# mjmyt/drone_path_planning_python

Measured on AMD Instinct MI355X. Metric: minimum-snap trajectories/sec (N drones × M segments, order 7) at 1/2/4/8 MI355X, higher is better.
Workload: dtype f64

## Files before the change

drone_path_planning_python_amd/csrc/msnap_api.hip:

```cpp
#include <cstdarg>
#include <cstdio>
#include <cstdlib>
#include <cstring>
#include <initializer_list>
#include <new>

#include "msnap_internal.h"

namespace msnap {

int record_hip_error(msnap_ctx *ctx, hipError_t e, const char *what) {
  if (ctx) snprintf(ctx->hip_err, sizeof(ctx->hip_err), "%s: %s", what, hipGetErrorString(e));
  return MSNAP_EHIP;
}

int handover_form(const msnap_ctx *ctx, const void *ptr, const void *pos, int n, int n_samples) {
  if (!ptr) return 0;
  for (const auto &h : ctx->handover)
    if (h.ptr == ptr) return (h.pos == pos && h.n == n && h.s == n_samples) ? h.form : 0;
  return 0;
}

bool stream_is_capturing(const msnap_ctx *ctx) {
  hipStreamCaptureStatus st = hipStreamCaptureStatusNone;
// ... 42 lines not shown
  do {                                                            \
    const int rc__ = (check);                                     \
    if (rc__) return rc__ == msnap::kNoWork ? MSNAP_OK : rc__;    \
    MSNAP_HIP(ctx, hipSetDevice((ctx)->device));                  \
  } while (0)

struct Region {
  const void *in;
  void *out;
  size_t bytes;
};
static Region upload(const void *h, size_t bytes) { return {h, nullptr, bytes}; }
static Region download(void *h, size_t bytes) { return {nullptr, h, bytes}; }

struct DevPtr {
  void *p;
  template <class T>
  operator T *() const { return static_cast<T *>(p); }
};

template <size_t K, class Launch>
static int staged(msnap_ctx *ctx, const Region (&r)[K], Launch &&launch) {
  size_t off[K], total = 0;
  for (size_t k = 0; k < K; ++k) {
    off[k] = total;
    total += r[k].bytes ? (r[k].bytes + 255) & ~(size_t)255 : 256;
  }
  int rc = ensure(ctx, ctx->host_stage, total);
  if (rc) return rc;
  DevPtr d[K];
  for (size_t k = 0; k < K; ++k) {
    d[k].p = (char *)ctx->host_stage.p + off[k];
    if (r[k].in && r[k].bytes)
      MSNAP_HIP(ctx, hipMemcpyAsync(d[k].p, r[k].in, r[k].bytes, hipMemcpyHostToDevice, ctx->stream));
  }
  if ((rc = launch(d))) return rc;
  for (size_t k = 0; k < K; ++k)
    if (r[k].out && r[k].bytes)
      MSNAP_HIP(ctx, hipMemcpyAsync(r[k].out, d[k].p, r[k].bytes, hipMemcpyDeviceToHost, ctx->stream));
  MSNAP_HIP(ctx, hipStreamSynchronize(ctx->stream));
  return MSNAP_OK;
}

static size_t coef_bytes(const msnap_ctx *ctx, int n_drones, int n_seg) {
  return (size_t)n_drones * n_seg * 4 * (ctx->order + 1) * 8;
}
static size_t dur_bytes(int n_drones, int n_seg) { return (size_t)n_drones * n_seg * 8; }

struct OptionName {
  const char *name, *env;
};
static const OptionName kOptions[] = {
    {"solve_grid_waves", "MSNAP_SOLVE_GRID_WAVES"}, {"gemm_grid_waves", "MSNAP_GEMM_GRID_WAVES"},
    {"twist_max_drones", "MSNAP_TWIST_MAX_DRONES"}, {"no_twist", "MSNAP_NO_TWIST"},
    {"collide_waves_per_cu", "MSNAP_COLLIDE_WAVES_PER_CU"}, {"pipe_chunk_mb", "MSNAP_PIPE_CHUNK_MB"},
    {"collide_sample_parts", "MSNAP_COLLIDE_SAMPLE_PARTS"}, {"no_twin", "MSNAP_NO_TWIN"}, {"no_grid_sample", "MSNAP_NO_GRID_SAMPLE"}, {"gemm_stream_waves_per_cu", "MSNAP_GEMM_STREAM_WAVES_PER_CU"}, {"mesh_waves_per_cu", "MSNAP_MESH_WAVES_PER_CU"}, {"collide_no_cull", "MSNAP_COLLIDE_NO_CULL"}, {"collide_cull_min_drones", "MSNAP_COLLIDE_CULL_MIN_DRONES"}, {"collide_cull_mode", "MSNAP_COLLIDE_CULL_MODE"}, {"twin_max_drones", "MSNAP_TWIN_MAX_DRONES"},
};

void note_kernel(msnap_ctx *ctx, const char *fmt, ...) {
  va_list ap;
  va_start(ap, fmt);
  vsnprintf(ctx->last_kernel, sizeof(ctx->last_kernel), fmt, ap);
  va_end(ap);
}

static bool option_is_read_only(const char *name) { return !strncmp(name, "collide_last_", 13); }

static int *option_slot(msnap_ctx *ctx, const char *name) {
  if (!strcmp(name, "solve_grid_waves")) return &ctx->solve_grid_waves;
  if (!strcmp(name, "gemm_grid_waves")) return &ctx->gemm_grid_waves;
  if (!strcmp(name, "twist_max_drones")) return &ctx->twist_max_drones;
  if (!strcmp(name, "no_twist")) return &ctx->no_twist;
  if (!strcmp(name, "no_twin")) return &ctx->no_twin;
  if (!strcmp(name, "no_grid_sample")) return &ctx->no_grid_sample;
  if (!strcmp(name, "gemm_stream_waves_per_cu")) return &ctx->gemm_stream_waves_per_cu;
  if (!strcmp(name, "mesh_waves_per_cu")) return &ctx->mesh_waves_per_cu;
  if (!strcmp(name, "twin_max_drones")) return &ctx->twin_max_drones;
  if (!strcmp(name, "collide_waves_per_cu")) return &ctx->collide_waves_per_cu;
  if (!strcmp(name, "collide_sample_parts")) return &ctx->collide_sample_parts;
  if (!strcmp(name, "collide_no_sym")) return &ctx->collide_no_sym;
  if (!strcmp(name, "collide_no_cull")) return &ctx->collide_no_cull;
  if (!strcmp(name, "collide_cull_min_drones")) return &ctx->collide_cull_min_drones;
  if (!strcmp(name, "collide_cull_mode")) return &ctx->collide_cull_mode;
  if (!strcmp(name, "collide_last_cull")) return &ctx->collide_last_cull;
  if (!strcmp(name, "collide_last_shares")) return &ctx->collide_last_shares;
  if (!strcmp(name, "collide_last_sym")) return &ctx->collide_last_sym;
  if (!strcmp(name, "collide_last_handover")) return &ctx->collide_last_handover;
  if (!strcmp(name, "own_stream_priority")) return &ctx->own_stream_priority;
  return nullptr;
}

}

using namespace msnap;

extern "C" {

int msnap_version(void) { return MSNAP_VERSION_NUM; }

const char *msnap_strerror(int code) {
  switch (code) {
    case MSNAP_OK: return "ok";
    case MSNAP_EINVAL: return "invalid argument";
    case MSNAP_EHIP: return "HIP runtime error (see msnap_last_hip_error)";
    case MSNAP_EORDER: return "unsupported polynomial order (7 or 9)";
    case MSNAP_ESEGMENTS: return "segment count out of range for this context, or not the prepared grid's";
    case MSNAP_ENOMEM: return "out of memory";
    case MSNAP_ENODEVICE: return "no usable gfx950 device";
    case MSNAP_ENOGRID: return "no time grid prepared on this context (msnap_grid_prepare)";
    case MSNAP_ECAPTURE: return "a scratch buffer would have to grow during stream capture: run the call once outside the capture first";
    default: return "unknown msnap error";
  }
}

const char *msnap_last_hip_error(const msnap_ctx *ctx) { return ctx ? ctx->hip_err : ""; }

const char *msnap_last_kernel(const msnap_ctx *ctx) { return ctx ? ctx->last_kernel : ""; }

int msnap_create(msnap_ctx **out, int device_id, int order, int max_segments) {
  if (!out) return MSNAP_EINVAL;
  *out = nullptr;
  if (order != 7 && order != 9) return MSNAP_EORDER;
  if (max_segments < 1) return MSNAP_ESEGMENTS;
  int ndev = 0;
  if (hipGetDeviceCount(&ndev) != hipSuccess || ndev <= 0) return MSNAP_ENODEVICE;
// ... 70 lines not shown
  }
  if (bytes) *bytes = freed;
  return rc;
}

int msnap_set_stream(msnap_ctx *ctx, void *hip_stream) {
  if (!ctx) return MSNAP_EINVAL;
  ctx->stream = reinterpret_cast<hipStream_t>(hip_stream);
  return MSNAP_OK;
}

int msnap_use_own_stream(msnap_ctx *ctx) {
  if (!ctx) return MSNAP_EINVAL;
  ctx->stream = ctx->own_stream;
  return MSNAP_OK;
}

int msnap_set_option(msnap_ctx *ctx, const char *name, long value) {
  if (!ctx || !name || value < 0 || value > (1L << 30)) return MSNAP_EINVAL;
  if (!strcmp(name, "pipe_chunk_mb")) {
    ctx->pipe_chunk_bytes = (size_t)(value > 0 ? value : 64) << 20;
    return MSNAP_OK;
  }
  if (!strcmp(name, "own_stream_priority")) {
    if (value > 2) return MSNAP_EINVAL;
    MSNAP_HIP(ctx, hipSetDevice(ctx->device));
    int least = 0, greatest = 0;
    MSNAP_HIP(ctx, hipDeviceGetStreamPriorityRange(&least, &greatest));
    hipStream_t fresh = nullptr;
    MSNAP_HIP(ctx, hipStreamCreateWithPriority(&fresh, hipStreamNonBlocking,
                                               value == 1 ? least : value == 2 ? greatest : 0));
    const bool current = ctx->stream == ctx->own_stream;
    if (ctx->own_stream) {
      (void)hipStreamSynchronize(ctx->own_stream);
      (void)hipStreamDestroy(ctx->own_stream);
    }
    ctx->own_stream = fresh;
    if (current) ctx->stream = fresh;
    ctx->own_stream_priority = (int)value;
    return MSNAP_OK;
  }
  if (!strcmp(name, "mesh_count_tests")) {
    MSNAP_HIP(ctx, hipSetDevice(ctx->device));
    MSNAP_HIP(ctx, hipStreamSynchronize(ctx->stream));
    if (value && !ctx->mesh_tests) MSNAP_HIP(ctx, hipMalloc(&ctx->mesh_tests, 8));
    if (ctx->mesh_tests) MSNAP_HIP(ctx, hipMemset(ctx->mesh_tests, 0, 8));
    if (!value && ctx->mesh_tests) {
      (void)hipFree(ctx->mesh_tests);
      ctx->mesh_tests = nullptr;
    }
    return MSNAP_OK;
  }
  if (option_is_read_only(name)) return MSNAP_EINVAL;
  int *slot = option_slot(ctx, name);
  if (!slot) return MSNAP_EINVAL;
  *slot = (int)value;
  return MSNAP_OK;
}

int msnap_get_option(const msnap_ctx *ctx, const char *name, long *value) {
  if (!ctx || !name || !value) return MSNAP_EINVAL;
  if (!strcmp(name, "pipe_chunk_mb")) {
    *value = (long)(ctx->pipe_chunk_bytes >> 20);
    return MSNAP_OK;
  }
  if (!strcmp(name, "mesh_count_tests")) {
    unsigned long long n = 0;
    if (ctx->mesh_tests) {
      if (stream_is_capturing(ctx)) return MSNAP_ECAPTURE;
      if (hipSetDevice(ctx->device) != hipSuccess || hipStreamSynchronize(ctx->stream) != hipSuccess ||
          hipMemcpy(&n, ctx->mesh_tests, 8, hipMemcpyDeviceToHost) != hipSuccess)
        return MSNAP_EHIP;
    }
    *value = (long)n;
    return MSNAP_OK;
  }
  if (!strcmp(name, "collide_last_group_pairs") || !strcmp(name, "collide_last_survivors") ||
      !strcmp(name, "collide_last_by_groups") || !strcmp(name, "collide_last_pairs_evaluated")) {
    int32_t shares = ctx->collide_last_shares, groups = 0;
    const bool culled = ctx->collide_last_cull && ctx->collide_meta;
    if (culled) {
      if (stream_is_capturing(ctx)) return MSNAP_ECAPTURE;
      if (hipSetDevice(ctx->device) != hipSuccess || hipStreamSynchronize(ctx->stream) != hipSuccess ||
          hipMemcpy(&shares, ctx->collide_meta + MSNAP_COLLIDE_META_SHARES, sizeof shares, hipMemcpyDeviceToHost) != hipSuccess ||
          hipMemcpy(&groups, ctx->collide_meta + MSNAP_COLLIDE_META_GROUPS, sizeof groups, hipMemcpyDeviceToHost) != hipSuccess)
        return MSNAP_EHIP;
    }
    const bool by_groups = culled && (ctx->collide_last_by_groups == 1 || (ctx->collide_last_by_groups == 2 && groups <= (1 << 18)));
    if (!strcmp(name, "collide_last_group_pairs")) *value = groups;
    else if (!strcmp(name, "collide_last_survivors")) *value = shares;
    else if (!strcmp(name, "collide_last_by_groups")) *value = by_groups ? 1 : 0;
    else *value = !culled ? -1 : by_groups ? (long)groups * 64 : (long)shares * 1024;
    return MSNAP_OK;
  }
  const int *slot = option_slot(const_cast<msnap_ctx *>(ctx), name);
  if (!slot) return MSNAP_EINVAL;
  *value = *slot;
  return MSNAP_OK;
}

int msnap_host_alloc(void **ptr, size_t bytes) {
  if (!ptr) return MSNAP_EINVAL;
  *ptr = nullptr;
  if (bytes == 0) return MSNAP_OK;
  hipError_t e = hipHostMalloc(ptr, bytes, hipHostMallocDefault);
  if (e != hipSuccess) {
// ... 578 lines not shown
```

drone_path_planning_python_amd/csrc/msnap_internal.h:

```cpp
#pragma once

#include <hip/hip_runtime.h>
#include <stddef.h>
#include <stdint.h>

#include "../../include/msnap.h"

#define MSNAP_VERSION_NUM 300
#define MSNAP_COLLIDE_META_SHARES 128
#define MSNAP_COLLIDE_META_GROUPS 132

namespace msnap {

constexpr int kWave = 64;
constexpr int kAxes = 4;
constexpr int kDronesPerWave = 16;
constexpr size_t kMaxLdsBytes = 160 * 1024;

inline size_t solve_scratch_words(int khalf, int n_seg) {
  const size_t nu = (size_t)khalf - 1;
  const size_t M = (size_t)n_seg;
  const size_t knots = M > 0 ? M - 1 : 0;
  return 16 * M + 16 * nu * nu * knots + 64 * nu * knots;
}
inline size_t solve_input_words(int n_seg) { return (size_t)16 * (n_seg + 1) * 5; }

template <int N>
__device__ __forceinline__ void wait_vmcnt() {
  static_assert(N >= 0 && N < 64, "6-bit vmcnt field");
  asm volatile("s_waitcnt vmcnt(%0)" ::"n"(N) : "memory");
}

__device__ __forceinline__ void lds_barrier() { asm volatile("s_waitcnt lgkmcnt(0)\n\ts_barrier" ::: "memory"); }

struct DevBuf {
  void *p = nullptr;
  size_t cap = 0;
  bool in_graph = false;
};
struct RetiredBuf {
  void *p;
  size_t cap;
  RetiredBuf *next;
};

}

struct msnap_ctx {
  int device = 0;
  int order = 7;
  int khalf = 4;
  int max_segments = 0;
  int n_cu = 256;
  hipStream_t own_stream = nullptr;
  hipStream_t stream = nullptr;
  hipEvent_t ev0 = nullptr, ev1 = nullptr;
  msnap::DevBuf scratch;
  msnap::DevBuf host_stage;
  msnap::DevBuf collide_work;
  msnap::DevBuf limits_work;
  hipStream_t pipe_stream[2] = {nullptr, nullptr};
  hipEvent_t pipe_start = nullptr;
  msnap::DevBuf pipe[2][5];
  size_t pipe_chunk_bytes = 64u << 20;
  void *bounce = nullptr;
  size_t bounce_cap = 0;
  msnap::DevBuf grid_t, grid_wp, grid_op, grid_dur, grid_status, grid_frag;
  int grid_seg = 0;
  int grid_ready = 0;
  int no_twist = 0;
  int gemm_stream_waves_per_cu = 0;
  int no_grid_sample = 0;
  int no_twin = 0;
  int twin_max_drones = 0;
  int twist_max_drones = 0;
  int solve_grid_waves = 0;
  int gemm_grid_waves = 0;
  void *mesh_tests = nullptr;
  int collide_waves_per_cu = 0;
  int collide_sample_parts = 0;
  int collide_no_sym = 0;
  int collide_no_cull = 0;
  int collide_cull_mode = 0;
  int collide_cull_min_drones = 0;
  int collide_last_cull = 0;
  int collide_last_shares = 0;
  const int32_t *collide_meta = nullptr;
  int collide_last_by_groups = 0;
  int collide_last_n = 0;
  const void *blist_clean = nullptr;
  int blist_clean_n = 0;
  unsigned long long *cull_hint = nullptr;
  struct Handover {
    const void *ptr = nullptr;
    const void *pos = nullptr;
    int n = 0, s = 0, form = 0;
  } handover[8];
  int handover_next = 0;
  int collide_last_sym = 0;
  int collide_last_handover = 0;
  int mesh_waves_per_cu = 0;
  int own_stream_priority = 0;
  msnap::RetiredBuf *retired = nullptr;
  char hip_err[256] = {0};
  char last_kernel[96] = {0};
};

namespace msnap {

int record_hip_error(msnap_ctx *ctx, hipError_t e, const char *what);
int ensure(msnap_ctx *ctx, DevBuf &b, size_t bytes);
bool stream_is_capturing(const msnap_ctx *ctx);
int handover_form(const msnap_ctx *ctx, const void *ptr, const void *pos, int n, int n_samples);
bool collide_counts_by_groups(const msnap_ctx *ctx, int n_drones, int shares_surviving, int group_pairs_surviving);

void note_kernel(msnap_ctx *ctx, const char *fmt, ...) __attribute__((format(printf, 2, 3)));

#define MSNAP_HIP(ctx, call)                                         \
  do {                                                               \
    hipError_t e__ = (call);                                         \
    if (e__ != hipSuccess) return msnap::record_hip_error(ctx, e__, #call); \
  } while (0)

int launch_solve(msnap_ctx *ctx, int n_drones, int n_seg, const double *wp, const double *t,
                 int shared_times, double *coef, double *dur, int32_t *status);
int launch_pack(msnap_ctx *ctx, int n_drones, int n_seg, const double *coef, const double *dur,
                float *out);
int launch_formation_transform(msnap_ctx *ctx, int n_poses, int n_offsets, const double *rb_pose,
// ... 53 lines not shown
```

drone_path_planning_python_amd/csrc/msnap_solve.hip:

```cpp
#include "msnap_consts.h"
#include <cstdlib>

#include "msnap_internal.h"

namespace msnap {

__device__ __forceinline__ constexpr int sidx(int r, int c) {
  return r * (r + 1) / 2 + c;
}

__device__ __forceinline__ double rcp64(double v) {
  double r = __builtin_amdgcn_rcp(v);
  double e = __builtin_fma(-v, r, 1.0);
  r = __builtin_fma(r, e, r);
  e = __builtin_fma(-v, r, 1.0);
  r = __builtin_fma(r, e, r);
  return r;
}

__device__ __forceinline__ bool finite64(double v) { return __builtin_isfinite(v); }

template <int K>
struct Sweep {
  static constexpr int NU = K - 1;
// ... 247 lines not shown
        "s"(mask), "v"(keep[0]), "v"(keep[1]), "v"(keep[2]), "v"(keep[3]), "v"(keep[4]), "v"(keep[5]), "v"(keep[6]), \
        "v"(keep[7])                                                                                               \
      : "vcc")
template <int STAGE>
__device__ __forceinline__ void quad_stage(uint32_t (&a)[8], uint32_t (&b)[8], unsigned long long bit) {
  uint32_t na[8], nb[8];
  const unsigned long long nbit = ~bit;
  if constexpr (STAGE == 1) {
    MSNAP_QSTAGE("[1,0,3,2]", nb, a, b, bit);
    MSNAP_QSTAGE("[1,0,3,2]", na, b, a, nbit);
  } else {
    MSNAP_QSTAGE("[2,3,0,1]", nb, a, b, bit);
    MSNAP_QSTAGE("[2,3,0,1]", na, b, a, nbit);
  }
#pragma unroll
  for (int k = 0; k < 8; ++k) {
    a[k] = na[k];
    b[k] = nb[k];
  }
}
#undef MSNAP_QSTAGE
#undef MSNAP_QCND

__device__ __forceinline__ void store_quad8_at(double *__restrict__ blk, int a, const double (&c)[8], bool bad) {
  double p[8];
#pragma unroll
  for (int k = 0; k < 8; ++k) p[k] = c[k];
  if (__builtin_expect(__builtin_amdgcn_ballot_w64(bad) != 0, 0)) {
    asm volatile("" ::: "memory");
#pragma unroll
    for (int k = 0; k < 8; ++k) p[k] = bad ? __builtin_nan("") : p[k];
  }
  auto lo = [](double v) { return (uint32_t)__double2loint(v); };
  auto hi = [](double v) { return (uint32_t)__double2hiint(v); };
  uint32_t A[8] = {lo(p[0]), hi(p[0]), lo(p[1]), hi(p[1]), lo(p[4]), hi(p[4]), lo(p[5]), hi(p[5])};
  uint32_t B[8] = {lo(p[2]), hi(p[2]), lo(p[3]), hi(p[3]), lo(p[6]), hi(p[6]), lo(p[7]), hi(p[7])};
  quad_stage<1>(A, B, __builtin_amdgcn_ballot_w64((a & 1) != 0));
  uint32_t A2[8] = {A[0], A[1], A[2], A[3], B[0], B[1], B[2], B[3]};
  uint32_t B2[8] = {A[4], A[5], A[6], A[7], B[4], B[5], B[6], B[7]};
  quad_stage<2>(A2, B2, __builtin_amdgcn_ballot_w64((a & 2) != 0));
  uint4 *o = reinterpret_cast<uint4 *>(blk + a * 2);
  o[0] = make_uint4(A2[0], A2[1], A2[2], A2[3]);
  o[4] = make_uint4(A2[4], A2[5], A2[6], A2[7]);
  o[8] = make_uint4(B2[0], B2[1], B2[2], B2[3]);
  o[12] = make_uint4(B2[4], B2[5], B2[6], B2[7]);
}

__device__ __forceinline__ void store_segment_quad8(double *__restrict__ seg_base, size_t drone_stride,
                                                    int nvalid, int lane, const double (&c)[8], bool bad) {
  const int dl = lane >> 2;
  store_quad8_at(seg_base + (size_t)(dl < nvalid ? dl : nvalid - 1) * drone_stride, lane & 3, c, bad);
}

template <int MAXCNT = 0>
__device__ __forceinline__ void store_durations(const double *sTraw, int shared_times, int tpitch, int M,
                                                int nvalid, int lane, double *__restrict__ dur_tile) {
  const int cnt = nvalid * M;
  auto one = [&](int e) {
    if (e < cnt) {
      const int dl = e / M;
      const int i = e - dl * M;
      const double *lt = sTraw + (shared_times ? 0 : dl * tpitch);
      dur_tile[e] = lt[i + 1] - lt[i];
    }
  };
  if constexpr (MAXCNT > 0) {
#pragma unroll
    for (int e0 = 0; e0 < MAXCNT; e0 += kWave) one(e0 + lane);
  } else {
    for (int e0 = 0; e0 < cnt; e0 += kWave) one(e0 + lane);
  }
}

__device__ __forceinline__ int drone_status(bool nonfinite, bool badtime, bool singular) {
  int flags = (nonfinite ? 4 : 0) | (badtime ? 2 : 0) | (singular ? 1 : 0);
  flags |= __shfl_xor(flags, 1);
  flags |= __shfl_xor(flags, 2);
  return (flags & 4) ? MSNAP_ST_NONFINITE : (flags & 2) ? MSNAP_ST_TIMES : (flags & 1) ? MSNAP_ST_SINGULAR : MSNAP_ST_OK;
}

__device__ __forceinline__ void stage_inputs(const double *__restrict__ wp, const double *__restrict__ tt,
                                             int shared_times, int tile, int nvalid, int wpitch, int tpitch,
                                             double *sWraw, double *sTraw, int lane) {
  const double2 *wsrc = reinterpret_cast<const double2 *>(wp + (size_t)tile * kDronesPerWave * wpitch);
  double2 *wdst = reinterpret_cast<double2 *>(sWraw);
  const int wcnt = nvalid * wpitch / 2;
  const double *tsrc = shared_times ? tt : tt + (size_t)tile * kDronesPerWave * tpitch;
  const int tcnt = shared_times ? tpitch : nvalid * tpitch;
  constexpr int UW = 8, UT = 4;
  for (int e0 = 0, f0 = 0; e0 < wcnt || f0 < tcnt; e0 += UW * kWave, f0 += UT * kWave) {
    double2 vw[UW];
    double vt[UT];
#pragma unroll
    for (int u = 0; u < UW; ++u) {
      const int e = e0 + u * kWave + lane;
      vw[u] = wsrc[e < wcnt ? e : wcnt - 1];
    }
#pragma unroll
    for (int u = 0; u < UT; ++u) {
      const int f = f0 + u * kWave + lane;
      vt[u] = tsrc[f < tcnt ? f : tcnt - 1];
    }
#pragma unroll
    for (int u = 0; u < UW; ++u) asm volatile("" : "+v"(vw[u].x), "+v"(vw[u].y));
#pragma unroll
    for (int u = 0; u < UT; ++u) asm volatile("" : "+v"(vt[u]));
#pragma unroll
    for (int u = 0; u < UW; ++u) {
      const int e = e0 + u * kWave + lane;
      if (e < wcnt) wdst[e] = vw[u];
    }
#pragma unroll
    for (int u = 0; u < UT; ++u) {
      const int f = f0 + u * kWave + lane;
      if (f < tcnt) sTraw[f] = vt[u];
    }
  }
}

template <int MAXM>
struct StageRegs {
  static constexpr int UW = (MAXM + 2) / 2;
  static constexpr int UT = (MAXM + 4) / 4;
// ... 777 lines not shown
        __builtin_amdgcn_sched_barrier(0);
        const int nx = next < ntiles ? next : ntiles - 1;
        twin_stage_load<M>(wp, tt, shared_times, nx, tile_valid(nx), lane, pre);
      }
      const bool own = !kAsym || it <= nL || side != 0;
      double u[NU];
      if (it >= 1) {
        const double2 *gsl = reinterpret_cast<const double2 *>(sG + (it - 1) * kSlotWords + blk * kAxes);
#pragma unroll
        for (int r = 0; r < NU; ++r) {
          const double2 g01 = gsl[r * (kWave / 2)], g23 = gsl[r * (kWave / 2) + 1];
          double v = (it <= ZL) ? sZ[((it >= 1 ? it - 1 : 0) * NU + r) * kWave + lane] : zreg[it >= 1 ? it - 1 : 0][r];
          v = __builtin_fma(-g01.x, un[0], v);
          v = __builtin_fma(-g01.y, un[1], v);
          v = __builtin_fma(-g23.x, un[2], v);
          if constexpr (NU == 4) v = __builtin_fma(-g23.y, un[3], v);
          u[r] = v;
        }
      } else {
#pragma unroll
        for (int r = 0; r < NU; ++r) u[r] = zero_or_nan;
      }
      double ua[NU], ub[NU];
#pragma unroll
      for (int r = 0; r < NU; ++r) {
        ua[r] = side ? dsg[r] * un[r] : u[r];
        ub[r] = side ? dsg[r] * u[r] : un[r];
      }
      const double wa = side ? wreg[it + 1] : wreg[it];
      const double wb = side ? wreg[it] : wreg[it + 1];
      double xi = xreg[it];
      asm volatile("" : "+v"(xi));
      double c[NC];
      recover_segment<K>(wa, wb - wa, xi, ua, ub, c);
      if (side == 0 && it == 0 && t0 != 0.0) taylor_shift<NC>(c, -t0);
      if (own) {
        if constexpr (NC == 10) store_twin_coalesced(sTr, blkp, lane, plan, c);
        else store_quad8_at(blkp, a, c, false);
      }
      blkp += blkstep;
#pragma unroll
      for (int r = 0; r < NU; ++r) un[r] = own ? u[r] : un[r];
    }
  }
}

constexpr int kTwistDrones = 8;
constexpr int kTwistFenceHalf = 9;

#ifdef MSNAP_TOOLS_TIMELINE
__device__ unsigned long long g_timeline[1024 * 32];
#define MSNAP_TL(k)                                                                       \
  do {                                                                                    \
    const int it__ = (tl_tile - (int)blockIdx.x) / (int)gridDim.x;                        \
    if (lane == 0 && blockIdx.x < 1024 && it__ < 2) {                                     \
      g_timeline[blockIdx.x * 32 + 16 * it__ + 2 * (k)] = wall_clock64();                 \
      g_timeline[blockIdx.x * 32 + 16 * it__ + 2 * (k) + 1] = clock64();                  \
    }                                                                                     \
  } while (0)
#else
#define MSNAP_TL(k) do { } while (0)
#endif

template <int K, int MAXH, int M>
__global__ void __launch_bounds__(kWave)
solve_kernel_twist(const double *__restrict__ wp, const double *__restrict__ tt, int shared_times,
                   int N, double *__restrict__ coef, double *__restrict__ dur,
                   int32_t *__restrict__ status, int ntiles) {
  using SW = Sweep<K>;
  constexpr int NU = SW::NU, NC = SW::NC, NS = SW::NS;
  constexpr int nL = (M - 2) / 2, nR = (M - 2) - nL;
  static_assert(M >= 2 && MAXH == nR, "MAXH is the knot count of the longer side");
  constexpr int HA = MAXH > 0 ? MAXH : 1;

  extern __shared__ __attribute__((aligned(16))) double lds[];

  const int lane = threadIdx.x;
  const int a = lane & 3;
  const int side = (lane >> 2) & 1;
  const int dl = lane >> 3;
  constexpr int wpitch = (M + 1) * 4;
  constexpr int tpitch = M + 1;
  const int mside = side ? nR : nL;
  double *sWraw = lds;
  double *sTraw = sWraw + kTwistDrones * wpitch;
  double dsg[NU];
#pragma unroll
  for (int r = 0; r < NU; ++r) dsg[r] = (r & 1) ? 1.0 : -1.0;

  const int tile = blockIdx.x;
  (void)ntiles;
  {
#ifdef MSNAP_TOOLS_TIMELINE
    const int tl_tile = tile;
#endif
    MSNAP_TL(0);
    const int d_raw = tile * kTwistDrones + dl;
    const bool live = d_raw < N;
    const int d = live ? d_raw : N - 1;
    const int left = N - tile * kTwistDrones;
    const int nvalid = left < kTwistDrones ? left : kTwistDrones;

    {
      const double2 *wsrc = reinterpret_cast<const double2 *>(wp + (size_t)tile * kTwistDrones * wpitch);
      double2 *wdst = reinterpret_cast<double2 *>(sWraw);
      const int wcnt = nvalid * wpitch / 2;
      const double *tsrc = shared_times ? tt : tt + (size_t)tile * kTwistDrones * tpitch;
      const int tcnt = shared_times ? tpitch : nvalid * tpitch;
      constexpr int UW = (kTwistDrones * wpitch / 2 + kWave - 1) / kWave;
      constexpr int UT = (kTwistDrones * tpitch + kWave - 1) / kWave;
      double2 vw[UW];
      double vt[UT];
#pragma unroll
      for (int u = 0; u < UW; ++u) {
        const int e = u * kWave + lane;
        vw[u] = wsrc[e < wcnt ? e : wcnt - 1];
      }
#pragma unroll
      for (int u = 0; u < UT; ++u) {
        const int f = u * kWave + lane;
        vt[u] = tsrc[f < tcnt ? f : tcnt - 1];
      }
#pragma unroll
      for (int u = 0; u < UW; ++u) asm volatile("" : "+v"(vw[u].x), "+v"(vw[u].y));
#pragma unroll
      for (int u = 0; u < UT; ++u) asm volatile("" : "+v"(vt[u]));
#pragma unroll
      for (int u = 0; u < UW; ++u) {
        const int e = u * kWave + lane;
        if (e < wcnt) wdst[e] = vw[u];
      }
#pragma unroll
      for (int u = 0; u < UT; ++u) {
        const int f = u * kWave + lane;
        if (f < tcnt) sTraw[f] = vt[u];
      }
    }
    __syncthreads();
    MSNAP_TL(1);

    const int dloc = live ? dl : (N - 1 - tile * kTwistDrones);
    const double *lw = sWraw + dloc * wpitch + a;
    const double *lt = sTraw + (shared_times ? 0 : dloc * tpitch);
    auto Wown = [&](int i) -> double { return lw[(side ? M - i : i) * 4]; };
    auto Town = [&](int i) -> double {
      const int j = side ? M - 1 - i : i;
      return lt[j + 1] - lt[j];
    };

    constexpr bool kZReg = MAXH * NU < 3 * kTwistFenceHalf;
    double wreg[HA + 2], xreg[HA + 1], zreg[kZReg ? HA : 1][NU];
    double *sZ = sTraw + kTwistDrones * tpitch + lane;
    double Greg[HA][NU][NU];
    const double t0 = lt[0];
    wreg[0] = Wown(0);
    wreg[1] = Wown(1);
    const double T0 = Town(0);
    const double T0q = side ? T0 : T0 - t0;
    bool nonfinite = !(finite64(t0) & finite64(T0) & finite64(wreg[0]) & finite64(wreg[1]));
    bool badtime = !(T0 > 0.0) | !(T0q > 0.0) | (t0 < 0.0);
    xreg[0] = rcp64(T0q);
    SW sw;
    sw.init(xreg[0], wreg[1] - wreg[0]);

    double xpc[SW::PM + 1], dwc = 0.0;
    auto ahead = [&](int it, double (&xp)[SW::PM + 1], double &dw) {
      wreg[it + 1] = Wown(it + 1);
      const double Tit = Town(it);
      nonfinite |= !finite64(Tit) | !finite64(wreg[it + 1]);
      badtime |= !(Tit > 0.0);
      xreg[it] = rcp64(Tit);
      SW::powers(xreg[it], xp);
      dw = wreg[it + 1] - wreg[it];
    };
    if (MAXH >= 1) ahead(1, xpc, dwc);
    bool singular = false;
    auto knot_step = [&](int it) {
      double G[NU][NU], z[NU];
      typename SW::Knot k;
      SW::knot_geom_xp(xpc, dwc, sw.E, sw.re, k);
      const bool ok = sw.chain(k, G, z);
      singular |= !ok & (it <= mside);
#pragma unroll
      for (int e = 0; e < NS; ++e) sw.E[e] = k.E[e];
#pragma unroll
      for (int r = 0; r < NU; ++r) {
        sw.re[r] = k.re[r];
        if constexpr (kZReg) zreg[it - 1][r] = z[r];
        else sZ[((it - 1) * NU + r) * kWave] = z[r];
#pragma unroll
        for (int c = 0; c < NU; ++c) Greg[it - 1][r][c] = G[r][c];
      }
    };
#pragma unroll
    for (int it = 1; it <= MAXH; ++it) {
      if (it < MAXH) {
        double xpn[SW::PM + 1], dwn;
        ahead(it + 1, xpn, dwn);
        knot_step(it);
        dwc = dwn;
#pragma unroll
        for (int q = 0; q <= SW::PM; ++q) xpc[q] = xpn[q];
        if constexpr (MAXH * NU >= 3 * kTwistFenceHalf) __builtin_amdgcn_sched_barrier(0);
      } else if (nL == nR) {
        knot_step(it);
      } else {
        double E0[NS], G0[NS], r0[NU], z0[NU];
#pragma unroll
        for (int e = 0; e < NS; ++e) { E0[e] = sw.E[e]; G0[e] = sw.OtG[e]; }
#pragma unroll
        for (int r = 0; r < NU; ++r) { r0[r] = sw.re[r]; z0[r] = sw.Otz[r]; }
        knot_step(it);
#pragma unroll
        for (int e = 0; e < NS; ++e) { sw.E[e] = side ? sw.E[e] : E0[e]; sw.OtG[e] = side ? sw.OtG[e] : G0[e]; }
#pragma unroll
        for (int r = 0; r < NU; ++r) { sw.re[r] = side ? sw.re[r] : r0[r]; sw.Otz[r] = side ? sw.Otz[r] : z0[r]; }
      }
    }

    MSNAP_TL(2);
    double Sm[NS], um[NU];
#pragma unroll
    for (int r = 0; r < NU; ++r) {
      const double q = sw.re[r] + sw.Otz[r];
      um[r] = -q - dsg[r] * __shfl_xor(q, 4);
#pragma unroll
      for (int c = 0; c <= r; ++c) {
        const double p = sw.E[sidx(r, c)] - sw.OtG[sidx(r, c)];
        Sm[sidx(r, c)] = p + (dsg[r] * dsg[c]) * __shfl_xor(p, 4);
      }
    }
    {
      double dinv[NU];
      singular |= SW::ldl_factor(Sm, dinv);
      SW::ldl_solve(Sm, dinv, um);
    }

    const int gsh = lane & ~7;
    const bool f_nonfinite = ((__ballot(nonfinite) >> gsh) & 0xFFull) != 0;
    const bool f_time = ((__ballot(badtime) >> gsh) & 0xFFull) != 0;
    const bool f_sing = ((__ballot(singular) >> gsh) & 0xFFull) != 0;
    const int st = f_nonfinite ? MSNAP_ST_NONFINITE : f_time ? MSNAP_ST_TIMES : f_sing ? MSNAP_ST_SINGULAR : MSNAP_ST_OK;
    if (live && (lane & 7) == 0) status[d] = st;
    const bool bad = st != 0;

    MSNAP_TL(3);
    const double qnan = __builtin_nan("");
    const double zero_or_nan = bad ? qnan : 0.0;
#pragma unroll
    for (int i = 0; i < MAXH + 2; ++i) wreg[i] = bad ? qnan : wreg[i];
    double un[NU];
#pragma unroll
    for (int r = 0; r < NU; ++r) un[r] = bad ? qnan : um[r];
#pragma unroll
    for (int it = MAXH; it >= 0; --it) {
      if (it <= nL || side) {
        double u[NU];
        if (it >= 1) {
#pragma unroll
          for (int r = 0; r < NU; ++r) {
            double v;
            if constexpr (kZReg) v = zreg[it >= 1 ? it - 1 : 0][r];
            else v = sZ[((it >= 1 ? it - 1 : 0) * NU + r) * kWave];
#pragma unroll
            for (int c = 0; c < NU; ++c) v = __builtin_fma(-Greg[it >= 1 ? it - 1 : 0][r][c], un[c], v);
            u[r] = v;
          }
        } else {
#pragma unroll
          for (int r = 0; r < NU; ++r) u[r] = zero_or_nan;
        }
        double ua[NU], ub[NU];
#pragma unroll
        for (int r = 0; r < NU; ++r) {
          ua[r] = side ? dsg[r] * un[r] : u[r];
          ub[r] = side ? dsg[r] * u[r] : un[r];
        }
        const double wa = side ? wreg[it + 1] : wreg[it];
        const double wb = side ? wreg[it] : wreg[it + 1];
        double c[NC];
        recover_segment<K>(wa, wb - wa, xreg[it], ua, ub, c);
        if (side == 0 && it == 0 && t0 != 0.0) taylor_shift<NC>(c, -t0);
        const int seg = side ? M - 1 - it : it;
        {
          double *o = coef + (((size_t)d * M + seg) * 4 + a) * NC;
#pragma unroll
          for (int m = 0; m < NC; m += 2) *reinterpret_cast<double2 *>(o + m) = make_double2(c[m], c[m + 1]);
        }
#pragma unroll
        for (int r = 0; r < NU; ++r) un[r] = u[r];
      }
      if constexpr (MAXH * NU >= 3 * kTwistFenceHalf) __builtin_amdgcn_sched_barrier(0);
    }
    __builtin_amdgcn_sched_barrier(0);
    store_durations<kTwistDrones * M>(sTraw, shared_times, tpitch, M, nvalid, lane, dur + (size_t)tile * kTwistDrones * M);
    MSNAP_TL(4);
  }
}

constexpr int kTwistMaxSeg = 24;
constexpr int kTwistMaxSeg9 = 12;

constexpr int kTwinMaxSeg = 20;
constexpr int kTwinMaxSeg7 = 20;
constexpr int kRegMaxSeg = 10;
constexpr int kRegMaxSeg2 = 20;

template <int K>
static int launch_solve_k(msnap_ctx *ctx, int N, int M, const double *wp, const double *t, int shared,
                          double *coef, double *dur, int32_t *status) {
  const int ntiles = (N + kDronesPerWave - 1) / kDronesPerWave;
  const size_t tr_bytes = (size_t)K * kTrPitch * 16;
  const bool twin_ok = (M >= 4 && M <= (K == 5 ? kTwinMaxSeg : kTwinMaxSeg7) && !ctx->no_twin &&
                        (ctx->twin_max_drones > 0 ? N <= ctx->twin_max_drones
                                                   : (K == 5 || N <= ctx->n_cu * 256 || M > kRegMaxSeg)));
  const int twist_max = ctx->twist_max_drones > 0 ? ctx->twist_max_drones
                                                  : ctx->n_cu * (twin_ok ? 1 : 4) * kTwistDrones;
  if (M >= 2 && M <= (K == 4 ? kTwistMaxSeg : kTwistMaxSeg9) && N <= twist_max && !ctx->no_twist) {
    const int nt8 = (N + kTwistDrones - 1) / kTwistDrones;
    const int nR = (M - 2) - (M - 2) / 2;
    const size_t lds_bytes = ((size_t)kTwistDrones * (M + 1) * 5 + (size_t)64 * (K - 1) * nR) * sizeof(double);
#define MSNAP_TWIST_EXACT(MM)                                                                          \
  case MM:                                                                                             \
    note_kernel(ctx, "msnap::solve_kernel_twist<%d, %d, %d>", K, (MM - 2) - (MM - 2) / 2, MM);         \
    hipLaunchKernelGGL((solve_kernel_twist<K, (MM - 2) - (MM - 2) / 2, MM>), dim3(nt8), dim3(kWave),   \
                       lds_bytes, ctx->stream, wp, t, shared, N, coef, dur, status, nt8);             \
    break;
    if constexpr (K == 4) {
      switch (M) {
        MSNAP_TWIST_EXACT(2) MSNAP_TWIST_EXACT(3) MSNAP_TWIST_EXACT(4) MSNAP_TWIST_EXACT(5)
        MSNAP_TWIST_EXACT(6) MSNAP_TWIST_EXACT(7) MSNAP_TWIST_EXACT(8) MSNAP_TWIST_EXACT(9)
        MSNAP_TWIST_EXACT(10) MSNAP_TWIST_EXACT(11) MSNAP_TWIST_EXACT(12) MSNAP_TWIST_EXACT(13)
        MSNAP_TWIST_EXACT(14) MSNAP_TWIST_EXACT(15) MSNAP_TWIST_EXACT(16) MSNAP_TWIST_EXACT(17)
        MSNAP_TWIST_EXACT(18) MSNAP_TWIST_EXACT(19) MSNAP_TWIST_EXACT(20) MSNAP_TWIST_EXACT(21)
        MSNAP_TWIST_EXACT(22) MSNAP_TWIST_EXACT(23) MSNAP_TWIST_EXACT(24)
        default: return MSNAP_EINVAL;
      }
    } else {
      switch (M) {
        MSNAP_TWIST_EXACT(2) MSNAP_TWIST_EXACT(3) MSNAP_TWIST_EXACT(4) MSNAP_TWIST_EXACT(5)
        MSNAP_TWIST_EXACT(6) MSNAP_TWIST_EXACT(7) MSNAP_TWIST_EXACT(8) MSNAP_TWIST_EXACT(9)
        MSNAP_TWIST_EXACT(10) MSNAP_TWIST_EXACT(11) MSNAP_TWIST_EXACT(12)
        default: return MSNAP_EINVAL;
      }
    }
#undef MSNAP_TWIST_EXACT
    MSNAP_HIP(ctx, hipGetLastError());
    return MSNAP_OK;
  }
  if (twin_ok) {
    const int nt8 = (N + kTwinDrones - 1) / kTwinDrones;
    int grid = ctx->n_cu * 8 * 8;
    if (ctx->solve_grid_waves > 0) grid = ctx->solve_grid_waves;
    if (grid > nt8) grid = nt8;
#define MSNAP_TWIN(MM)                                                                                            \
  case MM:                                                                                                        \
    note_kernel(ctx, "msnap::solve_kernel_twin<%d, %d>", K, MM);                                                  \
    hipLaunchKernelGGL((solve_kernel_twin<K, MM>), dim3(grid), dim3(kWave), twin_lds_bytes(K, MM), ctx->stream,   \
                       wp, t, shared, N, coef, dur, status, nt8);                                                 \
    break;
    if constexpr (K == 5) {
      switch (M) {
        MSNAP_TWIN(4) MSNAP_TWIN(5) MSNAP_TWIN(6) MSNAP_TWIN(7) MSNAP_TWIN(8) MSNAP_TWIN(9) MSNAP_TWIN(10)
        MSNAP_TWIN(11) MSNAP_TWIN(12) MSNAP_TWIN(13) MSNAP_TWIN(14) MSNAP_TWIN(15) MSNAP_TWIN(16) MSNAP_TWIN(17)
        MSNAP_TWIN(18) MSNAP_TWIN(19) MSNAP_TWIN(20)
        default: return MSNAP_EINVAL;
      }
    } else {
      switch (M) {
        MSNAP_TWIN(4) MSNAP_TWIN(5) MSNAP_TWIN(6) MSNAP_TWIN(7) MSNAP_TWIN(8) MSNAP_TWIN(9) MSNAP_TWIN(10)
        MSNAP_TWIN(11) MSNAP_TWIN(12) MSNAP_TWIN(13) MSNAP_TWIN(14) MSNAP_TWIN(15) MSNAP_TWIN(16) MSNAP_TWIN(17)
        MSNAP_TWIN(18) MSNAP_TWIN(19) MSNAP_TWIN(20)
        default: return MSNAP_EINVAL;
      }
    }
#undef MSNAP_TWIN
    MSNAP_HIP(ctx, hipGetLastError());
    return MSNAP_OK;
  }
  if (M >= 2 && M <= kRegMaxSeg2) {
    const size_t nu = K - 1;
    const size_t in_bytes = solve_input_words(M) * sizeof(double);
    const size_t lds_bytes = (in_bytes > tr_bytes ? in_bytes : tr_bytes) +
                             16 * nu * nu * (size_t)(M > 2 ? M - 2 : 0) * sizeof(double);
    const bool two_per_simd = (K <= 4 && M <= kRegMaxSeg);
    int grid = ctx->n_cu * (two_per_simd ? 8 : 4) * 8;
    if (ctx->solve_grid_waves > 0) grid = ctx->solve_grid_waves;
    if (grid > ntiles) grid = ntiles;
    note_kernel(ctx, "msnap::solve_kernel_reg<%d, %d>", K, M <= kRegMaxSeg ? kRegMaxSeg : kRegMaxSeg2);
    if (M <= kRegMaxSeg)
      hipLaunchKernelGGL((solve_kernel_reg<K, kRegMaxSeg>), dim3(grid), dim3(kWave), lds_bytes, ctx->stream,
                         wp, t, shared, N, M, coef, dur, status, ntiles);
    else
      hipLaunchKernelGGL((solve_kernel_reg<K, kRegMaxSeg2>), dim3(grid), dim3(kWave), lds_bytes, ctx->stream,
                         wp, t, shared, N, M, coef, dur, status, ntiles);
    MSNAP_HIP(ctx, hipGetLastError());
    return MSNAP_OK;
  }
  const size_t words = solve_scratch_words(K, M);
// ... 50 lines not shown
```

Baseline: 58.94 million.

## Split twist solve back-substitution across multiple waves per tile for small drone counts

The twist solve kernel now runs with 1, 2 or 4 waves per tile. Each wave redundantly runs the forward sweep, then writes only its own chunk of the back-substitution segments, with a separate LDS slice per wave. Cooperative loads and duration stores are also spread over all threads. The wave count is picked automatically when there are too few tiles to fill the CUs, or set through a new option. The aim is to use idle CUs and shorten per-tile latency at small N, at the cost of redundant sweep work and more LDS and register pressure per block.

```diff
diff --git a/drone_path_planning_python_amd/csrc/msnap_api.hip b/drone_path_planning_python_amd/csrc/msnap_api.hip
--- a/drone_path_planning_python_amd/csrc/msnap_api.hip
+++ b/drone_path_planning_python_amd/csrc/msnap_api.hip
@@ -118,7 +118,7 @@
 };
 static const OptionName kOptions[] = {
     {"solve_grid_waves", "MSNAP_SOLVE_GRID_WAVES"}, {"gemm_grid_waves", "MSNAP_GEMM_GRID_WAVES"},
-    {"twist_max_drones", "MSNAP_TWIST_MAX_DRONES"}, {"no_twist", "MSNAP_NO_TWIST"},
+    {"twist_max_drones", "MSNAP_TWIST_MAX_DRONES"}, {"no_twist", "MSNAP_NO_TWIST"}, {"twist_waves", "MSNAP_TWIST_WAVES"},
     {"collide_waves_per_cu", "MSNAP_COLLIDE_WAVES_PER_CU"}, {"pipe_chunk_mb", "MSNAP_PIPE_CHUNK_MB"},
     {"collide_sample_parts", "MSNAP_COLLIDE_SAMPLE_PARTS"}, {"no_twin", "MSNAP_NO_TWIN"}, {"no_grid_sample", "MSNAP_NO_GRID_SAMPLE"}, {"gemm_stream_waves_per_cu", "MSNAP_GEMM_STREAM_WAVES_PER_CU"}, {"mesh_waves_per_cu", "MSNAP_MESH_WAVES_PER_CU"}, {"collide_no_cull", "MSNAP_COLLIDE_NO_CULL"}, {"collide_cull_min_drones", "MSNAP_COLLIDE_CULL_MIN_DRONES"}, {"collide_cull_mode", "MSNAP_COLLIDE_CULL_MODE"}, {"twin_max_drones", "MSNAP_TWIN_MAX_DRONES"},
 };
@@ -137,6 +137,7 @@
   if (!strcmp(name, "gemm_grid_waves")) return &ctx->gemm_grid_waves;
   if (!strcmp(name, "twist_max_drones")) return &ctx->twist_max_drones;
   if (!strcmp(name, "no_twist")) return &ctx->no_twist;
+  if (!strcmp(name, "twist_waves")) return &ctx->twist_waves;
   if (!strcmp(name, "no_twin")) return &ctx->no_twin;
   if (!strcmp(name, "no_grid_sample")) return &ctx->no_grid_sample;
   if (!strcmp(name, "gemm_stream_waves_per_cu")) return &ctx->gemm_stream_waves_per_cu;
@@ -313,6 +314,7 @@
     return MSNAP_OK;
   }
   if (option_is_read_only(name)) return MSNAP_EINVAL;
+  if (!strcmp(name, "twist_waves") && value != 0 && value != 1 && value != 2 && value != 4) return MSNAP_EINVAL;
   int *slot = option_slot(ctx, name);
   if (!slot) return MSNAP_EINVAL;
   *slot = (int)value;
diff --git a/drone_path_planning_python_amd/csrc/msnap_internal.h b/drone_path_planning_python_amd/csrc/msnap_internal.h
--- a/drone_path_planning_python_amd/csrc/msnap_internal.h
+++ b/drone_path_planning_python_amd/csrc/msnap_internal.h
@@ -74,6 +74,7 @@
   int no_twin = 0;
   int twin_max_drones = 0;
   int twist_max_drones = 0;
+  int twist_waves = 0;
   int solve_grid_waves = 0;
   int gemm_grid_waves = 0;
   void *mesh_tests = nullptr;
diff --git a/drone_path_planning_python_amd/csrc/msnap_solve.hip b/drone_path_planning_python_amd/csrc/msnap_solve.hip
--- a/drone_path_planning_python_amd/csrc/msnap_solve.hip
+++ b/drone_path_planning_python_amd/csrc/msnap_solve.hip
@@ -323,7 +323,7 @@
   store_quad8_at(seg_base + (size_t)(dl < nvalid ? dl : nvalid - 1) * drone_stride, lane & 3, c, bad);
 }
 
-template <int MAXCNT = 0>
+template <int MAXCNT = 0, int STRIDE = kWave>
 __device__ __forceinline__ void store_durations(const double *sTraw, int shared_times, int tpitch, int M,
                                                 int nvalid, int lane, double *__restrict__ dur_tile) {
   const int cnt = nvalid * M;
@@ -337,9 +337,9 @@
   };
   if constexpr (MAXCNT > 0) {
 #pragma unroll
-    for (int e0 = 0; e0 < MAXCNT; e0 += kWave) one(e0 + lane);
+    for (int e0 = 0; e0 < MAXCNT; e0 += STRIDE) one(e0 + lane);
   } else {
-    for (int e0 = 0; e0 < cnt; e0 += kWave) one(e0 + lane);
+    for (int e0 = 0; e0 < cnt; e0 += STRIDE) one(e0 + lane);
   }
 }
 
@@ -1223,21 +1223,26 @@
 __device__ unsigned long long g_timeline[1024 * 32];
 #define MSNAP_TL(k)                                                                       \
   do {                                                                                    \
-    const int it__ = (tl_tile - (int)blockIdx.x) / (int)gridDim.x;                        \
-    if (lane == 0 && blockIdx.x < 1024 && it__ < 2) {                                     \
-      g_timeline[blockIdx.x * 32 + 16 * it__ + 2 * (k)] = wall_clock64();                 \
-      g_timeline[blockIdx.x * 32 + 16 * it__ + 2 * (k) + 1] = clock64();                  \
+    const int row__ = (int)blockIdx.x * NW + wave;                                        \
+    if (lane == 0 && row__ < 1024) {                                                      \
+      g_timeline[row__ * 32 + 2 * (k)] = wall_clock64();                                  \
+      g_timeline[row__ * 32 + 2 * (k) + 1] = clock64();                                   \
     }                                                                                     \
   } while (0)
 #else
 #define MSNAP_TL(k) do { } while (0)
 #endif
 
-template <int K, int MAXH, int M>
-__global__ void __launch_bounds__(kWave)
+template <int S, int NW>
+__device__ __forceinline__ constexpr int twist_chunk_lo(int w) {
+  return w * (S / NW) + (w > NW - S % NW ? w - (NW - S % NW) : 0);
+}
+template <int K, int MAXH, int M, int NW>
+__global__ void __launch_bounds__(kWave * NW)
 solve_kernel_twist(const double *__restrict__ wp, const double *__restrict__ tt, int shared_times,
                    int N, double *__restrict__ coef, double *__restrict__ dur,
-                   int32_t *__restrict__ status, int ntiles) {
+                   int32_t *__restrict__ status) {
+  static_assert(NW == 1 || NW == 2 || NW == 4, "one, two or four waves per tile");
   using SW = Sweep<K>;
   constexpr int NU = SW::NU, NC = SW::NC, NS = SW::NS;
   constexpr int nL = (M - 2) / 2, nR = (M - 2) - nL;
@@ -1246,7 +1251,9 @@
 
   extern __shared__ __attribute__((aligned(16))) double lds[];
 
-  const int lane = threadIdx.x;
+  const int tid = threadIdx.x;
+  const int lane = NW > 1 ? tid & (kWave - 1) : tid;
+  const int wave = NW > 1 ? __builtin_amdgcn_readfirstlane(tid / kWave) : 0;
   const int a = lane & 3;
   const int side = (lane >> 2) & 1;
   const int dl = lane >> 3;
@@ -1260,11 +1267,7 @@
   for (int r = 0; r < NU; ++r) dsg[r] = (r & 1) ? 1.0 : -1.0;
 
   const int tile = blockIdx.x;
-  (void)ntiles;
   {
-#ifdef MSNAP_TOOLS_TIMELINE
-    const int tl_tile = tile;
-#endif
     MSNAP_TL(0);
     const int d_raw = tile * kTwistDrones + dl;
     const bool live = d_raw < N;
@@ -1273,23 +1276,24 @@
     const int nvalid = left < kTwistDrones ? left : kTwistDrones;
 
     {
+      constexpr int NT = kWave * NW;
       const double2 *wsrc = reinterpret_cast<const double2 *>(wp + (size_t)tile * kTwistDrones * wpitch);
       double2 *wdst = reinterpret_cast<double2 *>(sWraw);
       const int wcnt = nvalid * wpitch / 2;
       const double *tsrc = shared_times ? tt : tt + (size_t)tile * kTwistDrones * tpitch;
       const int tcnt = shared_times ? tpitch : nvalid * tpitch;
-      constexpr int UW = (kTwistDrones * wpitch / 2 + kWave - 1) / kWave;
-      constexpr int UT = (kTwistDrones * tpitch + kWave - 1) / kWave;
+      constexpr int UW = (kTwistDrones * wpitch / 2 + NT - 1) / NT;
+      constexpr int UT = (kTwistDrones * tpitch + NT - 1) / NT;
       double2 vw[UW];
       double vt[UT];
 #pragma unroll
       for (int u = 0; u < UW; ++u) {
-        const int e = u * kWave + lane;
+        const int e = u * NT + tid;
         vw[u] = wsrc[e < wcnt ? e : wcnt - 1];
       }
 #pragma unroll
       for (int u = 0; u < UT; ++u) {
-        const int f = u * kWave + lane;
+        const int f = u * NT + tid;
         vt[u] = tsrc[f < tcnt ? f : tcnt - 1];
       }
 #pragma unroll
@@ -1298,12 +1302,12 @@
       for (int u = 0; u < UT; ++u) asm volatile("" : "+v"(vt[u]));
 #pragma unroll
       for (int u = 0; u < UW; ++u) {
-        const int e = u * kWave + lane;
+        const int e = u * NT + tid;
         if (e < wcnt) wdst[e] = vw[u];
       }
 #pragma unroll
       for (int u = 0; u < UT; ++u) {
-        const int f = u * kWave + lane;
+        const int f = u * NT + tid;
         if (f < tcnt) sTraw[f] = vt[u];
       }
     }
@@ -1321,7 +1325,7 @@
 
     constexpr bool kZReg = MAXH * NU < 3 * kTwistFenceHalf;
     double wreg[HA + 2], xreg[HA + 1], zreg[kZReg ? HA : 1][NU];
-    double *sZ = sTraw + kTwistDrones * tpitch + lane;
+    double *sZ = sTraw + kTwistDrones * tpitch + wave * (HA * NU * kWave) + lane;
     double Greg[HA][NU][NU];
     const double t0 = lt[0];
     wreg[0] = Wown(0);
@@ -1412,10 +1416,11 @@
     const bool f_time = ((__ballot(badtime) >> gsh) & 0xFFull) != 0;
     const bool f_sing = ((__ballot(singular) >> gsh) & 0xFFull) != 0;
     const int st = f_nonfinite ? MSNAP_ST_NONFINITE : f_time ? MSNAP_ST_TIMES : f_sing ? MSNAP_ST_SINGULAR : MSNAP_ST_OK;
-    if (live && (lane & 7) == 0) status[d] = st;
+    if (live && (lane & 7) == 0 && wave == NW - 1) status[d] = st;
     const bool bad = st != 0;
 
     MSNAP_TL(3);
+    const int lo = twist_chunk_lo<MAXH + 1, NW>(wave), hi = twist_chunk_lo<MAXH + 1, NW>(wave + 1) - 1;
     const double qnan = __builtin_nan("");
     const double zero_or_nan = bad ? qnan : 0.0;
 #pragma unroll
@@ -1425,6 +1430,7 @@
     for (int r = 0; r < NU; ++r) un[r] = bad ? qnan : um[r];
 #pragma unroll
     for (int it = MAXH; it >= 0; --it) {
+      if (NW > 1 && (it < lo || hi < lo)) break;
       if (it <= nL || side) {
         double u[NU];
         if (it >= 1) {
@@ -1441,6 +1447,7 @@
 #pragma unroll
           for (int r = 0; r < NU; ++r) u[r] = zero_or_nan;
         }
+        if (NW == 1 || it <= hi) {
         double ua[NU], ub[NU];
 #pragma unroll
         for (int r = 0; r < NU; ++r) {
@@ -1458,13 +1465,15 @@
 #pragma unroll
           for (int m = 0; m < NC; m += 2) *reinterpret_cast<double2 *>(o + m) = make_double2(c[m], c[m + 1]);
         }
+        }
 #pragma unroll
         for (int r = 0; r < NU; ++r) un[r] = u[r];
       }
       if constexpr (MAXH * NU >= 3 * kTwistFenceHalf) __builtin_amdgcn_sched_barrier(0);
     }
     __builtin_amdgcn_sched_barrier(0);
-    store_durations<kTwistDrones * M>(sTraw, shared_times, tpitch, M, nvalid, lane, dur + (size_t)tile * kTwistDrones * M);
+    store_durations<kTwistDrones * M, kWave * NW>(sTraw, shared_times, tpitch, M, nvalid, tid,
+                                                  dur + (size_t)tile * kTwistDrones * M);
     MSNAP_TL(4);
   }
 }
@@ -1490,12 +1499,17 @@
   if (M >= 2 && M <= (K == 4 ? kTwistMaxSeg : kTwistMaxSeg9) && N <= twist_max && !ctx->no_twist) {
     const int nt8 = (N + kTwistDrones - 1) / kTwistDrones;
     const int nR = (M - 2) - (M - 2) / 2;
-    const size_t lds_bytes = ((size_t)kTwistDrones * (M + 1) * 5 + (size_t)64 * (K - 1) * nR) * sizeof(double);
+    const int nw = ctx->twist_waves > 0 ? ctx->twist_waves : nt8 * 4 <= ctx->n_cu ? 4 : nt8 * 2 <= ctx->n_cu ? 2 : 1;
+    const size_t lds_bytes = ((size_t)kTwistDrones * (M + 1) * 5 + (size_t)nw * 64 * (K - 1) * nR) * sizeof(double);
+#define MSNAP_TWIST_NW(MM, NWV)                                                                                    \
+  hipLaunchKernelGGL((solve_kernel_twist<K, (MM - 2) - (MM - 2) / 2, MM, NWV>), dim3(nt8), dim3(kWave * NWV),      \
+                     lds_bytes, ctx->stream, wp, t, shared, N, coef, dur, status)
 #define MSNAP_TWIST_EXACT(MM)                                                                          \
   case MM:                                                                                             \
     note_kernel(ctx, "msnap::solve_kernel_twist<%d, %d, %d>", K, (MM - 2) - (MM - 2) / 2, MM);         \
-    hipLaunchKernelGGL((solve_kernel_twist<K, (MM - 2) - (MM - 2) / 2, MM>), dim3(nt8), dim3(kWave),   \
-                       lds_bytes, ctx->stream, wp, t, shared, N, coef, dur, status, nt8);             \
+    if (nw == 4) MSNAP_TWIST_NW(MM, 4);                                                                \
+    else if (nw == 2) MSNAP_TWIST_NW(MM, 2);                                                           \
+    else MSNAP_TWIST_NW(MM, 1);                                                                        \
     break;
     if constexpr (K == 4) {
       switch (M) {
@@ -1516,6 +1530,7 @@
       }
     }
 #undef MSNAP_TWIST_EXACT
+#undef MSNAP_TWIST_NW
     MSNAP_HIP(ctx, hipGetLastError());
     return MSNAP_OK;
   }
```

New measurement: 60.57 million (median of 6 runs). 1.03x the previous value.
